# acoustid/acoustid-index

Measured on AMD Instinct MI355X. Metric: queries/sec + p50 /_search latency, 100M-fp index, 1k-hash queries, higher is better.
Workload: dtype u32

## Files before the change

acoustid-index_amd/csrc/fpx_qsearch.hpp:

```cpp
#pragma once
#include <hip/hip_runtime.h>

#include "fpx_internal.h"

namespace fpx {

#ifndef FPX_QS_WG
#define FPX_QS_WG 256
#endif
#ifndef FPX_QS_WAVES
#define FPX_QS_WAVES 4
#endif
#ifndef FPX_QS_REC_CAP
#define FPX_QS_REC_CAP 8192
#endif
#ifndef FPX_QS_FLOG2
#define FPX_QS_FLOG2 11
#endif
constexpr uint32_t QS_WG = FPX_QS_WG;
constexpr uint32_t QS_REC_CAP = FPX_QS_REC_CAP;
constexpr uint32_t QS_FLOG2 = FPX_QS_FLOG2;
constexpr uint32_t QS_TLOG2 = 8;
constexpr uint32_t QS_MAX_HASHES = QS_REC_CAP >= 8192u ? 4096u : 2048u;
constexpr uint32_t QS_MAX_ROUNDS = 32;
#ifndef FPX_QS_WORDS
#define FPX_QS_WORDS 12
#endif
#ifndef FPX_QS_CH
#define FPX_QS_CH 2
#endif
constexpr uint32_t QS_WORDS = FPX_QS_WORDS;
constexpr uint32_t QS_CH = FPX_QS_CH;
constexpr uint32_t QS_TASKS = (((size_t)2u << QS_FLOG2) + ((size_t)8u << QS_TLOG2)) / 8u;
constexpr uint32_t QS_TASK_WORDS = 8;
constexpr uint32_t QS_TASKS_FILT = QS_TASKS * 8u / 12u;
static_assert(QS_MAX_HASHES * 2u <= QS_REC_CAP, "the dedup set lives where the records will");
static_assert((QS_MAX_HASHES + QS_WG - 1u) / QS_WG <= QS_MAX_ROUNDS, "rounds per query");
static_assert(QS_WORDS % 4 == 0 && QS_WORDS <= 16, "the words are fetched in 16-byte pieces; a lane's masks of them are 16 bits");
#ifndef FPX_QS_DYN
#define FPX_QS_DYN 1
#endif
#ifndef FPX_QS_STAGGER
#define FPX_QS_STAGGER 1
#endif
constexpr uint32_t QS_STAGGER = FPX_QS_STAGGER;
#ifndef FPX_QS_WGS_PER_CU
#define FPX_QS_WGS_PER_CU 4
#endif
constexpr uint32_t QS_WGS_PER_CU = FPX_QS_WGS_PER_CU;
constexpr size_t QS_LDS_BYTES = ((size_t)QS_REC_CAP + 4u) * 4u + ((size_t)2u << QS_FLOG2) + ((size_t)8u << QS_TLOG2) + (size_t)SB_CAND * 8u;

struct QSearchArgs {
    const uint32_t* hashes_base; const uint64_t* offsets;
    const uint32_t* opts;
    uint32_t q_begin, q_end, sb;
    uint64_t* cands; uint64_t cand_cap;
    uint64_t* qcand; uint32_t* qcand_n;
    unsigned long long* counters;
    unsigned long long* stat_sets;
    unsigned long long* qstats;
    const uint32_t* cancel;
    const uint64_t* mem_tab; const uint32_t* mem_bucket; const uint32_t* mem_bits;
    unsigned int* next_q;
    uint32_t stagger;
    unsigned long long* redo; uint32_t redo_cap;
};

struct QSKernargs { QSearchArgs a; GroupArgs ga; };
typedef const __attribute__((address_space(4))) QSKernargs* qs_kargs_t;
__device__ __forceinline__ qs_kargs_t qs_cold_args()
{
    qs_kargs_t p = (qs_kargs_t)__builtin_amdgcn_kernarg_segment_ptr();
    asm volatile("" : "+s"(p));
    return p;
}

#define FPX_QS_OCC __attribute__((amdgpu_waves_per_eu(FPX_QS_WAVES)))
typedef uint32_t u32x3_t __attribute__((ext_vector_type(3)));
__device__ __forceinline__ uint3 gload_u3(const uint32_t* p)
{
    const u32x3_t v = *(const FPX_GLOBAL u32x3_t*)p;
    return make_uint3(v.x, v.y, v.z);
}
__device__ __forceinline__ uint32_t qs_cell(uint32_t doc) { return (doc ^ (doc >> QS_FLOG2)) & ((1u << QS_FLOG2) - 1u); }
__device__ __forceinline__ unsigned long long qs_task_list(const uint32_t* p, uint32_t chunk)
{
    return ((unsigned long long)p >> 2) | ((unsigned long long)chunk << 57) | (1ull << 63);
}
__device__ __forceinline__ unsigned long long qs_task_words(const uint32_t* p, uint32_t cnt, uint32_t second, uint32_t chunk)
{
    return ((unsigned long long)p >> 2) | ((unsigned long long)(cnt - 1u) << 46) | ((unsigned long long)(second & 0xFFu) << 49) | ((unsigned long long)chunk << 57);
}
__device__ __forceinline__ const uint32_t* qs_task_ptr(unsigned long long e) { return reinterpret_cast<const uint32_t*>((e & ((1ull << 46) - 1ull)) << 2); }
__device__ __forceinline__ uint32_t qs_word_cols(uint32_t pm, uint32_t dm, uint32_t j0, uint32_t cnt)
{
    uint32_t cols = 0, rest = pm, i = 0, w = 0;
    while (rest != 0u && w < j0 + cnt) {
        const uint32_t s = (uint32_t)__builtin_ctz(rest), span = 1u + ((dm >> i) & 1u);
        for (uint32_t t = 0; t < span; ++t, ++w) if (w >= j0 && w < j0 + cnt) cols |= s << (4u * (w - j0));
        ++i; rest &= rest - 1u;
    }
    return cols;
}

template <uint32_t K> __device__ __forceinline__ uint32_t qs_group_bcast(uint32_t v)
{
    return (uint32_t)__builtin_amdgcn_ds_swizzle((int)v, (int)((K << 5) | 0x18u));
}
template <uint32_t K> __device__ __forceinline__ uint32_t qs_from_sub0(uint32_t v)
{
    if constexpr (K == 0u) return v;
    else return (uint32_t)__builtin_amdgcn_update_dpp(0, (int)v, 0x110 | (int)K, 0xF, 0xF, true);
}
template <uint32_t K> __device__ __forceinline__ uint32_t qs_from_sub7(uint32_t v)
{
    if constexpr (K == 7u) return v;
    else return (uint32_t)__builtin_amdgcn_update_dpp(0, (int)v, 0x100 | (int)(7u - K), 0xF, 0xF, true);
}
template <uint32_t K> struct qs_idx { static constexpr uint32_t value = K; };
template <uint32_t K = 0, class F> __device__ __forceinline__ void qs_for8(F&& f)
{
    if constexpr (K < 8u) { f(qs_idx<K>{}); qs_for8<K + 1u>(f); }
}

#ifdef FPX_QS_PROF
#define QS_MARK(i) do { if (tid == 0) { const unsigned long long t_ = clock64(); atomicAdd(&qs_cold_args()->a.counters[CTR_HIST + (i)], t_ - t_prev); t_prev = t_; } } while (0)
#define QS_SUB0() do { if (tid == 0) t_sub = clock64(); } while (0)
#define QS_SUB(i) do { if (tid == 0) { const unsigned long long t_ = clock64(); atomicAdd(&qs_cold_args()->a.counters[CTR_HIST + (i)], t_ - t_sub); t_sub = t_; } } while (0)
#define QS_ARRIVED2(x, y) asm volatile("" :: "v"(x), "v"(y))
#define QS_ARRIVED4(x) asm volatile("" :: "v"((x)[0]), "v"((x)[1]), "v"((x)[2]), "v"((x)[3]))
#else
#define QS_MARK(i) do { } while (0)
#define QS_SUB0() do { } while (0)
#define QS_SUB(i) do { } while (0)
#define QS_ARRIVED2(x, y) do { } while (0)
#define QS_ARRIVED4(x) do { } while (0)
#endif
constexpr uint32_t QS_MAX_CLASSES = 32;
constexpr uint32_t QS_LIST_AHEAD = 8;
__device__ __forceinline__ uint32_t qs_class(uint32_t rec) { return mix32(rec) >> 27; }
static_assert(QS_MAX_CLASSES == 32u, "qs_class gives five bits");
constexpr uint32_t QS_LOW_CHUNK = 8;
template <int NS, bool QS, bool MEM, bool FILT, bool CLS, bool LOW = false, bool NEXT = false>
__device__ __forceinline__ void qs_body(const QSearchArgs& a, const GroupArgs& ga)
{
    static_assert(!NEXT || (!CLS && !LOW && !MEM), "a later group's walk: no doc classes, no low floors, no memory table (they ride on the first group's launch)");
    static_assert(!(CLS && FILT), "doc classes: the unfiltered walk only");
    static_assert(!LOW || (!CLS && QS_WG == 256u && QS_REC_CAP >= 512u && (QS_REC_CAP & (QS_REC_CAP - 1u)) == 0u),
                  "low floors: no doc classes; the sorted tail's scans are written for 256 lanes and a power-of-two array");
#ifdef FPX_QS_PROF
    unsigned long long t_prev = clock64(), t_sub = 0;
#endif
    constexpr uint32_t HVL = NS == 16 ? 2u : 3u;
    constexpr uint32_t T = 1u << QS_TLOG2, TMASK = T - 1u;
    extern __shared__ __align__(16) uint8_t qs_dyn[];
    uint32_t* const recs = reinterpret_cast<uint32_t*>(qs_dyn);
    uint32_t* const filter = recs + QS_REC_CAP + 4u;
    unsigned long long* const table = reinterpret_cast<unsigned long long*>(filter + (1u << (QS_FLOG2 - 1u)));
    unsigned long long* const tasks = reinterpret_cast<unsigned long long*>(filter);
    constexpr uint32_t TCAP = FILT ? QS_TASKS_FILT : QS_TASKS;
    uint32_t* const tcols = reinterpret_cast<uint32_t*>(tasks + QS_TASKS_FILT);
    uint64_t* const cbuf = reinterpret_cast<uint64_t*>(table + T);
    __shared__ uint32_t s_count, s_ntask, s_over_recs, s_seen_ones, s_cancel, s_claimed, s_full, s_ccnt, s_cshared, s_cbase_lo, s_cbase_hi;
    __shared__ unsigned long long wg_blocks, wg_docs, wg_probes, wg_reads;
    __shared__ uint32_t wg_h[HIST_SLOTS];
    __shared__ uint32_t s_first[FUSE_MAX], s_last[FUSE_MAX];
    __shared__ const uint32_t* s_ext[GROUP_CHUNKS];
    __shared__ uint32_t s_q2;
    __shared__ uint32_t s_dseg[FUSE_MAX];

    const uint32_t tid = threadIdx.x, lane = tid & 63u;
    const GroupDesc* g = &ga.g;
    uint32_t ent = a.q_begin + blockIdx.x;
    uint32_t q = ent, q_recs = 0u;
    uint32_t ncls = 1u;
    auto take_entry = [&]() {
        const unsigned long long e = qs_cold_args()->a.redo[ent];
        q = (uint32_t)__builtin_amdgcn_readfirstlane((int)(uint32_t)e); q_recs = (uint32_t)__builtin_amdgcn_readfirstlane((int)(uint32_t)(e >> 32));
        ncls = 1u;
        while ((unsigned long long)ncls * (QS_REC_CAP / 2u) < (unsigned long long)q_recs) ncls *= 2u;
    };
    if constexpr (CLS) take_entry();
    (void)q_recs;
    uint32_t qn = q + gridDim.x;
    uint32_t n, nn = 0u;
    uint64_t nq_lo = 0;
    const uint32_t* qh;
    if constexpr (CLS) {
        const uint64_t q_lo = a.offsets[q];
        n = (uint32_t)(a.offsets[q + 1] - q_lo);
        qh = a.hashes_base + q_lo;
        qn = 0xFFFFFFFFu;
    } else {
        const uint64_t q_lo = a.offsets[q];
        n = (uint32_t)(a.offsets[q + 1] - q_lo);
        qh = a.hashes_base + q_lo;
        if (qn < a.q_end) { nq_lo = a.offsets[qn]; nn = (uint32_t)(a.offsets[qn + 1] - nq_lo); }
    }
    {
        const qs_kargs_t ka = qs_cold_args();
        if (tid < FUSE_MAX) { s_first[tid] = ka->ga.g.first_hash[tid]; s_last[tid] = ka->ga.g.last_hash[tid]; }
        if (tid < GROUP_CHUNKS) s_ext[tid] = tid < ka->ga.g.nchunks ? ka->ga.g.ext_tab[tid] : nullptr;
        if (FILT && tid < FUSE_MAX) s_dseg[tid] = ka->ga.g.has_dead[tid] != 0u ? ka->ga.g.seg_index[tid] : 0xFFFFFFFFu;
    }
    const uint32_t gmin = (FILT || MEM) ? g->gmin : 0u;
    (void)gmin;
    uint32_t hq[2u * QS_CH];
    uint3 hd[QS_CH];
    auto line_of = [&](uint32_t h) -> const uint32_t* { return g->lines + (size_t)((h >> HVL) - g->line0) * GROUP_LINE_WORDS; };
    auto load_pair = [&](const uint32_t* qh_, uint32_t n_, uint32_t c, uint32_t& h0, uint32_t& h1) {
        const uint32_t i = c * QS_CH * QS_WG + tid;
        h0 = i < n_ ? gload_u32(qh_ + i) : 0u;
        h1 = i + QS_WG < n_ ? gload_u32(qh_ + i + QS_WG) : 0u;
    };
    auto issue_heads = [&](bool v0, bool v1) {
        hd[0] = gload_u3(v0 ? line_of(hq[0]) : g->lines);
        hd[1] = gload_u3(v1 ? line_of(hq[1]) : g->lines);
    };
    load_pair(qh, n, 0u, hq[0], hq[1]);
    load_pair(qh, n, 1u, hq[2], hq[3]);
    uint32_t c_host = 0u;
    unsigned long long c_dev = 0ull;
    auto ask_cancel = [&]() {
        const qs_kargs_t ka = qs_cold_args();
        const uint32_t* const cancel = ka->a.cancel;
        if (tid == 0u && cancel != nullptr) {
            if ((blockIdx.x & 63u) == 0u) c_host = __hip_atomic_load(cancel, __ATOMIC_RELAXED, __HIP_MEMORY_SCOPE_SYSTEM);
            c_dev = __hip_atomic_load(&ka->a.counters[CTR_CANCEL], __ATOMIC_RELAXED, __HIP_MEMORY_SCOPE_AGENT);
        }
    };
    ask_cancel();
  if (const uint32_t stagger = qs_cold_args()->a.stagger; !CLS && stagger != 0u && a.q_end - a.q_begin >= 4u * gridDim.x)
      for (uint32_t i = 0; i < ((blockIdx.x >> 8) & 3u) * stagger; ++i) __builtin_amdgcn_s_sleep(127);
  for (;;) {
    if constexpr (CLS) {
        if (ncls > QS_MAX_CLASSES) {
            if (tid == 0) atomicMax(&qs_cold_args()->a.counters[CTR_BINFAIL], 1ull);
            return;
        }
    }
    const uint32_t rounds = (n + QS_WG - 1u) / QS_WG, nchunks = (rounds + QS_CH - 1u) / QS_CH;
    uint32_t sbits = 8u;
    while ((1u << sbits) < 2u * n) ++sbits;
    if (tid < HIST_SLOTS) wg_h[tid] = 0u;
    for (uint32_t i = tid; i < (1u << sbits); i += QS_WG) recs[i] = 0xFFFFFFFFu;
    if (tid == 0) {
        s_count = 0u; s_ntask = 0u; s_over_recs = 0u; s_seen_ones = 0u; s_ccnt = 0u; s_cshared = 0u;
        wg_blocks = 0; wg_docs = 0; wg_probes = 0; wg_reads = 0;
        if (c_host != 0u) { atomicExch(&qs_cold_args()->a.counters[CTR_CANCEL], 1ull); c_dev = 1ull; }
        s_cancel = c_dev != 0ull ? 1u : 0u;
    }
    __syncthreads();
    if (s_cancel) return;
    QS_MARK(0);
    uint32_t vmask = 0u;
    uint32_t mmask = 0u;
    uint32_t nx[QS_CH] = {0u, 0u};
    for (uint32_t c = 0; c < nchunks; ++c) {
        uint32_t hc[QS_CH];
        uint32_t mb[QS_CH];
#pragma unroll
        for (uint32_t u = 0; u < QS_CH; ++u) hc[u] = c == 0u ? hq[u] : c == 1u ? hq[QS_CH + u] : nx[u];
        if (c != 0u) { QS_SUB0(); QS_ARRIVED2(hc[0], hc[1]); QS_SUB(6); }
        if (c != 0u && c + 1u < nchunks) load_pair(qh, n, c + 1u, nx[0], nx[1]);
        if constexpr (MEM) {
#pragma unroll
            for (uint32_t u = 0; u < QS_CH; ++u) {
                const uint32_t i = (c * QS_CH + u) * QS_WG + tid;
                mb[u] = (i < n && a.mem_bits != nullptr) ? gload_u32(a.mem_bits + ((hc[u] >> MEMTAB_FILTER_SHIFT) >> 5)) : 0xFFFFFFFFu;
            }
        }
#pragma unroll
        for (uint32_t u = 0; u < QS_CH; ++u) {
            const uint32_t i = (c * QS_CH + u) * QS_WG + tid;
            if (i >= n) continue;
            const uint32_t h = hc[u];
            bool dup;
            if (h == 0xFFFFFFFFu) dup = atomicExch(&s_seen_ones, 1u) != 0u;
            else {
                uint32_t slot = (h * 0x9E3779B1u) >> (32u - sbits);
                for (;;) {
                    const uint32_t old = atomicCAS(&recs[slot], 0xFFFFFFFFu, h);
                    if (old == 0xFFFFFFFFu) { dup = false; break; }
                    if (old == h) { dup = true; break; }
                    slot = (slot + 1u) & ((1u << sbits) - 1u);
                }
            }
            if (!dup && h >= g->win_lo && h <= g->win_hi) {
                vmask |= 1u << (c * QS_CH + u);
                if constexpr (MEM) mmask |= ((mb[u] >> ((h >> MEMTAB_FILTER_SHIFT) & 31u)) & 1u) << (c * QS_CH + u);
            }
        }
    }
    (void)mmask;
    __syncthreads();
    QS_MARK(1);

    const uint32_t cmask = ncls - 1u;
    (void)cmask;
    const bool has_next = qn < a.q_end;
    uint32_t q2 = 0u;
    bool has_q2 = false;
    uint64_t o2_lo = 0;
    uint32_t o2_hi = 0u;
  for (uint32_t cls = 0; cls < ncls; ++cls) {
    if constexpr (CLS) {
        if (cls != 0u) {
            __syncthreads();
            if (tid == 0) { s_count = 0u; s_ntask = 0u; }
            load_pair(qh, n, 0u, hq[0], hq[1]);
            __syncthreads();
        }
    }
    auto in_class = [&](uint32_t rec) -> bool { return (qs_class(rec) & cmask) == cls; };
    (void)in_class;
    const uint32_t active = g->active, nactive = (uint32_t)__popc(active);
    uint32_t my_blocks = 0, my_docs = 0, my_probes = 0, my_reads = 0;
    auto dead_in = [&](uint32_t s, uint32_t doc) -> bool {
        const uint32_t di = s_dseg[s];
        return di != 0xFFFFFFFFu && is_dead_seg(ga.segs[di], doc);
    };
    auto reserve_in = [&](uint32_t* counter, uint32_t cnt) -> uint32_t {
        const uint32_t incl = scan16(cnt);
        const uint32_t r0 = (uint32_t)__builtin_amdgcn_readlane((int)incl, 15), r1 = (uint32_t)__builtin_amdgcn_readlane((int)incl, 31),
                       r2 = (uint32_t)__builtin_amdgcn_readlane((int)incl, 47), r3 = (uint32_t)__builtin_amdgcn_readlane((int)incl, 63);
        const uint32_t total = r0 + r1 + r2 + r3;
        uint32_t wbase = 0;
        if (total != 0u) {
            if (lane == 0u) wbase = atomicAdd(counter, total);
            wbase = (uint32_t)__builtin_amdgcn_readfirstlane((int)wbase);
        }
        const uint32_t row = lane >> 4;
        return wbase + (row >= 1u ? r0 : 0u) + (row >= 2u ? r1 : 0u) + (row >= 3u ? r2 : 0u) + (incl - cnt);
    };
    auto reserve_both = [&](uint32_t cnt, uint32_t nt, uint32_t& tat) -> uint32_t {
        const uint32_t both = cnt | (nt << 16);
        const uint32_t incl = scan16(both);
        const uint32_t r0 = (uint32_t)__builtin_amdgcn_readlane((int)incl, 15), r1 = (uint32_t)__builtin_amdgcn_readlane((int)incl, 31),
                       r2 = (uint32_t)__builtin_amdgcn_readlane((int)incl, 47), r3 = (uint32_t)__builtin_amdgcn_readlane((int)incl, 63);
        const uint32_t total = r0 + r1 + r2 + r3;
        uint32_t rbase = 0, tbase = 0;
        if ((total & 0xFFFFu) != 0u) {
            if (lane == 0u) rbase = atomicAdd(&s_count, total & 0xFFFFu);
            rbase = (uint32_t)__builtin_amdgcn_readfirstlane((int)rbase);
        }
        if ((total >> 16) != 0u) {
            if (lane == 0u) tbase = atomicAdd(&s_ntask, total >> 16);
            tbase = (uint32_t)__builtin_amdgcn_readfirstlane((int)tbase);
        }
        const uint32_t row = lane >> 4;
        const uint32_t before = (row >= 1u ? r0 : 0u) + (row >= 2u ? r1 : 0u) + (row >= 3u ? r2 : 0u) + (incl - both);
        tat = tbase + (before >> 16);
        return rbase + (before & 0xFFFFu);
    };
    auto emit_at = [&](uint32_t km, const auto& d, uint32_t cnt, uint32_t pos) {
        constexpr uint32_t N = sizeof(d) / sizeof(uint32_t);
        if (cnt != 0u && pos + cnt > QS_REC_CAP) { s_over_recs = 1u; km = 0u; cnt = 0u; }
        const uint32_t first = cnt != 0u ? pos : QS_REC_CAP, sink = QS_REC_CAP - first;
#pragma unroll
        for (uint32_t j = N; j-- != 0u;) {
            const uint32_t last = (uint32_t)__popc(km & ((2u << j) - 1u)) - 1u;
            recs[first + min(last, sink)] = d[j];
        }
    };
    auto emit = [&](uint32_t km, const auto& d) {
        const uint32_t cnt = (uint32_t)__popc(km);
        emit_at(km, d, cnt, reserve_in(&s_count, cnt));
    };
    auto emit1 = [&](bool kp, uint32_t doc) {
        if constexpr (CLS) kp = kp && in_class(doc);
        const unsigned long long m = __ballot((int)kp);
        if (m == 0ull) return;
        uint32_t base = 0;
        if (lane == (uint32_t)__builtin_ctzll(m)) base = atomicAdd(&s_count, (uint32_t)__popcll(m));
        base = __shfl(base, (int)__builtin_ctzll(m));
        if (kp) {
            const uint32_t at = base + (uint32_t)__popcll(m & ((1ull << lane) - 1ull));
            if (at < QS_REC_CAP) recs[at] = doc; else s_over_recs = 1u;
        }
    };
    auto push_task = [&](unsigned long long e) {
        const uint32_t at = atomicAdd(&s_ntask, 1u);
        if (at < TCAP) tasks[at] = e; else s_over_recs = 1u;
    };

    auto words_of = [&](uint32_t h, uint3 head, bool valid, uint32_t (&gw)[QS_WORDS], uint32_t& hx, uint32_t& hy, uint32_t& ov) {
        const uint64_t bits = valid ? (((uint64_t)head.y << 32) | head.x) : 0ull;
        const uint32_t dfl = valid ? head.z : 0u;
        const uint32_t sh = (h & ((1u << HVL) - 1u)) * (uint32_t)NS;
        const uint32_t pm = (uint32_t)(bits >> sh) & ((1u << NS) - 1u);
        const uint32_t pos0 = (uint32_t)__popcll(bits & ((1ull << sh) - 1ull));
        const uint32_t k = (uint32_t)__popc(pm);
        const uint32_t dbl_before = pos0 >= 32u ? (uint32_t)__popc(dfl) : (uint32_t)__popc(dfl & ((1u << pos0) - 1u));
        const uint32_t dm = pos0 >= 32u ? 0u : ((dfl >> pos0) & ((1u << k) - 1u));
        const uint32_t nwords = k + (uint32_t)__popc(dm);
        const uint32_t n_line = (uint32_t)__popcll(bits) + (uint32_t)__popc(dfl);
        const uint32_t inl = n_line > GROUP_INLINE ? GROUP_INLINE - 1u : GROUP_INLINE;
        const uint32_t start = pos0 + dbl_before;
        const uint32_t mine = min(min(nwords, QS_WORDS), start < inl ? inl - start : 0u);
#pragma unroll
        for (uint32_t i = 0; i < QS_WORDS; ++i) gw[i] = 0xFFFFFFFFu;
        const uint32_t* lp = line_of(h) + 3u + start;
#pragma unroll
        for (uint32_t i = 0; i < QS_WORDS / 4; ++i) {
            if (mine > 4u * i) {
                const uint4 v = gload_u4_a4(lp + 4u * i);
                gw[4 * i] = v.x; gw[4 * i + 1] = v.y; gw[4 * i + 2] = v.z; gw[4 * i + 3] = v.w;
            }
        }
        ov = start + nwords > inl ? gload_u32(line_of(h) + (GROUP_LINE_WORDS - 1u)) : 0u;
        hx = start | (mine << 7) | (nwords << 11) | (inl << 17);
        hy = pm | (dm << 16);
    };
    auto probe = [&](uint32_t h, uint32_t hx, uint32_t hy, bool valid, uint32_t (&gw)[QS_WORDS], uint32_t ov) {
        if (valid) { my_probes += nactive; my_reads += 2u; }
        const uint32_t pm = hy & 0xFFFFu, dm = hy >> 16;
        const uint32_t start = hx & 127u, mine = (hx >> 7) & 15u, nwords = (hx >> 11) & 63u, inl = (hx >> 17) & 31u;
        uint32_t inr = active;
        if (h < g->lo_all || h > g->hi_all) {
            inr = 0u;
            uint32_t z = 0u;
            asm volatile("" : "+v"(z));
#pragma unroll
            for (uint32_t s = 0; s < NS; ++s) inr |= (h >= s_first[z + s] && h <= s_last[z + s]) ? (1u << s) : 0u;
        }
        if (!valid) inr = 0u;
        my_blocks += (uint32_t)__popc(inr & active & ~pm);
        uint32_t second = 0;
        for (uint32_t d = dm, t = 0; d != 0u; d &= d - 1u, ++t) second |= 1u << ((uint32_t)__builtin_ctz(d) + t + 1u);
        uint32_t negm = 0, gapm = 0;
#pragma unroll
        for (uint32_t j = 0; j < QS_WORDS; ++j) {
            const uint32_t word = gw[j];
            negm |= (word >> 31) << j;
            gapm |= (word == 0xFFFFFFFFu ? 1u : 0u) << j;
        }
        const uint32_t vm = (1u << mine) - 1u;
        uint32_t keep = vm & ~negm;
        uint32_t lmask = vm & negm & ~gapm;
        uint32_t dmask = 0;
        if constexpr (FILT) {
            uint32_t amask = 0;
            for (uint32_t r = pm, i = 0, w = 0; r != 0u && w < mine; r &= r - 1u, ++i) {
                const uint32_t s = (uint32_t)__builtin_ctz(r), span = 1u + ((dm >> i) & 1u), bits = ((1u << span) - 1u) << w;
                amask |= ((active >> s) & 1u) != 0u ? bits : 0u;
                dmask |= s_dseg[s] != 0xFFFFFFFFu ? bits : 0u;
                w += span;
            }
            keep &= amask; lmask &= amask;
        }
        my_docs += (uint32_t)__popc(keep);
        my_blocks += (uint32_t)__popc(keep & ~second);
        if constexpr (SCAN_HIST && (FPX_SH_BITS & 2)) my_probes += (uint32_t)__popc(keep & second) << 16;
        if constexpr (FILT) {
            for (uint32_t m = keep & dmask; m != 0u; m &= m - 1u) {
                const uint32_t j0 = (uint32_t)__builtin_ctz(m);
                uint32_t doc = 0;
#pragma unroll
                for (uint32_t j = 0; j < QS_WORDS; ++j) doc = j == j0 ? gw[j] : doc;
                if (dead_in(qs_word_cols(pm, dm, j0, 1u), gmin + doc)) keep &= ~(1u << j0);
            }
        }
        const uint32_t in_line = (nwords != mine && start + mine < inl) ? min(nwords - mine, inl - (start + mine)) : 0u;
        const uint32_t in_ext = nwords - mine - in_line;
        const uint32_t nt = (uint32_t)__popc(lmask) + (in_line + QS_TASK_WORDS - 1u) / QS_TASK_WORDS + (in_ext + QS_TASK_WORDS - 1u) / QS_TASK_WORDS;
        uint32_t tat;
        const uint32_t nrec = (uint32_t)__popc(keep);
        emit_at(keep, gw, nrec, reserve_both(nrec, nt, tat));
        if (nt != 0u) {
            if (tat + nt > TCAP) { s_over_recs = 1u; tat = TCAP; }
            auto put_task = [&](unsigned long long e) { if (tat < TCAP) tasks[tat] = e; ++tat; };
            auto put_words = [&](unsigned long long e, uint32_t j0, uint32_t c) {
                if constexpr (FILT) { if (tat < TCAP) tcols[tat] = qs_word_cols(pm, dm, j0, c); }
                put_task(e);
            };
            const uint32_t chunk = (h >> GROUP_CHUNK_LOG2) - g->chunk0;
            const uint32_t* ext = s_ext[chunk];
            uint32_t lm = lmask;
            while (lm != 0u) {
                const uint32_t j0 = (uint32_t)__builtin_ctz(lm);
                lm &= lm - 1u;
                uint32_t e = 0;
#pragma unroll
                for (uint32_t j = 0; j < QS_WORDS; ++j) e = j == j0 ? gw[j] : e;
                put_task(qs_task_list(ext + (e & 0x7FFFFFFFu), chunk) | (FILT ? ((unsigned long long)qs_word_cols(pm, dm, j0, 1u) << 46) : 0ull));
            }
            uint32_t j = mine;
            while (j < mine + in_line) {
                const uint32_t c = min(mine + in_line - j, QS_TASK_WORDS);
                put_words(qs_task_words(line_of(h) + 3u + start + j, c, second >> j, chunk), j, c);
                j += c;
            }
            if (j < nwords) {
                const uint32_t* ob = ext + ov;
                while (j < nwords) {
                    const uint32_t c = min(nwords - j, QS_TASK_WORDS);
                    put_words(qs_task_words(ob + (start + j - inl), c, second >> j, chunk), j, c);
                    j += c;
                }
                my_reads += 2u;
            }
        }
    };

    auto round_coop = [&](uint32_t h, bool valid) {
        const uint32_t sub = lane & 7u;
        uint32_t L[32];
        {
            const uint32_t li = valid ? (h >> HVL) - g->line0 : 0u;
            const uint8_t* const lb = reinterpret_cast<const uint8_t*>(g->lines) + 16u * sub;
            uint32_t lk[8];
            qs_for8([&](auto kc) { constexpr uint32_t k = decltype(kc)::value; lk[k] = qs_group_bcast<k>(li); });
            asm volatile("" : "+v"(lk[0]), "+v"(lk[1]), "+v"(lk[2]), "+v"(lk[3]), "+v"(lk[4]), "+v"(lk[5]), "+v"(lk[6]), "+v"(lk[7]));
            qs_for8([&](auto kc) {
                constexpr uint32_t k = decltype(kc)::value;
// ... 188 lines not shown
    QS_SUB0();
    QS_ARRIVED2(nn, (uint32_t)nq_lo); QS_SUB(11);
    uint32_t floor_v;
    {
        uint32_t qv = q;
        asm volatile("" : "+v"(qv));
        floor_v = gload_u32(qs_cold_args()->a.opts + (size_t)qv * 4u + 1u);
    }
    if (has_next) {
        const uint32_t* const qhn = a.hashes_base + nq_lo;
        load_pair(qhn, nn, 0u, hq[0], hq[1]);
        load_pair(qhn, nn, 1u, hq[2], hq[3]);
    }
    {
        uint32_t t_lo = 0;
        for (;;) {
            const uint32_t t_hi = min(s_ntask, TCAP);
            __syncthreads();
            if (t_lo >= t_hi) break;
            for (uint32_t t0 = t_lo; t0 < t_hi; t0 += QS_WG) {
                const bool has = t0 + tid < t_hi;
                const unsigned long long e = has ? tasks[t0 + tid] : 0ull;
                const bool is_list = has && (e >> 63) != 0ull;
                const uint32_t* p = qs_task_ptr(e);
                const uint32_t lcol = FILT ? (uint32_t)(e >> 46) & 15u : 0u;
                const uint32_t tc = (FILT && has && !is_list) ? tcols[t0 + tid] : 0u;
                uint32_t d[QS_TASK_WORDS];
#pragma unroll
                for (uint32_t j = 0; j < QS_TASK_WORDS; ++j) d[j] = 0xFFFFFFFFu;
                const uint32_t cnt = !has ? 0u : is_list ? 8u : ((uint32_t)(e >> 46) & 7u) + 1u;
#pragma unroll
                for (uint32_t i = 0; i < QS_TASK_WORDS / 4; ++i) {
                    if (cnt > 4u * i) {
                        const uint4 v = gload_u4_a4(p + 4u * i);
                        d[4 * i] = v.x; d[4 * i + 1] = v.y; d[4 * i + 2] = v.z; d[4 * i + 3] = v.w;
                    }
                }
                uint32_t km = 0, lm = 0;
                bool long_list = false;
                uint32_t eff = 0, Tl = 0, xin = 0;
                if (is_list) {
                    const uint32_t hdr = d[0];
                    eff = hdr & 0xFFFFu; Tl = (hdr >> 19) & 1u;
                    xin = min(eff, Tl ? 6u : 7u);
                    km = ((1u << xin) - 1u) << (1u + Tl);
                    my_blocks += (hdr >> 16) & 7u; my_docs += eff; my_reads += 2u;
                    hist_observe(wg_h, eff, (hdr >> 16) & 7u);
                    long_list = eff > xin;
                    if (long_list) my_reads += ((eff - xin + 31u) >> 5) * 2u;
                } else if (has) {
                    const uint32_t second = (uint32_t)(e >> 49) & 0xFFu;
                    uint32_t vm = (1u << cnt) - 1u, negm = 0, gapm = 0;
#pragma unroll
                    for (uint32_t j = 0; j < QS_TASK_WORDS; ++j) {
                        if constexpr (FILT) vm &= ~((((active >> ((tc >> (4u * j)) & 15u)) & 1u) ^ 1u) << j);
                        negm |= (d[j] >> 31) << j;
                        gapm |= (d[j] == 0xFFFFFFFFu ? 1u : 0u) << j;
                    }
                    km = vm & ~negm;
                    lm = vm & negm & ~gapm;
                    my_docs += (uint32_t)__popc(km); my_blocks += (uint32_t)__popc(km & ~second);
                    if constexpr (SCAN_HIST && (FPX_SH_BITS & 2)) my_probes += (uint32_t)__popc(km & second) << 16;
                }
                if constexpr (FILT) {
                    for (uint32_t m = km; m != 0u; m &= m - 1u) {
                        const uint32_t j0 = (uint32_t)__builtin_ctz(m);
                        const uint32_t s = is_list ? lcol : (tc >> (4u * j0)) & 15u;
                        if (s_dseg[s] == 0xFFFFFFFFu) continue;
                        uint32_t doc = 0;
#pragma unroll
                        for (uint32_t j = 0; j < QS_TASK_WORDS; ++j) doc = j == j0 ? d[j] : doc;
                        if (dead_in(s, gmin + doc)) km &= ~(1u << j0);
                    }
                }
                if constexpr (CLS) {
                    uint32_t cm = 0u;
#pragma unroll
                    for (uint32_t j = QS_TASK_WORDS; j-- != 0u;) cm = (cm << 1) | (in_class(d[j]) ? 1u : 0u);
                    km &= cm;
                }
                emit(km, d);
                while (lm != 0u) {
                    const uint32_t j0 = (uint32_t)__builtin_ctz(lm);
                    lm &= lm - 1u;
                    uint32_t w = 0;
#pragma unroll
                    for (uint32_t j = 0; j < QS_TASK_WORDS; ++j) w = j == j0 ? d[j] : w;
                    const uint32_t chunk = (uint32_t)(e >> 57) & 63u;
                    push_task(qs_task_list(s_ext[chunk] + (w & 0x7FFFFFFFu), chunk) | (FILT ? ((unsigned long long)((tc >> (4u * j0)) & 15u) << 46) : 0ull));
                }
                unsigned long long ml = __ballot((int)long_list);
                while (ml != 0ull) {
                    const int src = (int)__builtin_ctzll(ml);
                    ml &= ml - 1ull;
                    const uint32_t* list = reinterpret_cast<const uint32_t*>(((uint64_t)__shfl((uint32_t)((uint64_t)p >> 32), src) << 32) | __shfl((uint32_t)(uint64_t)p, src));
                    const uint32_t eff_s = __shfl(eff, src), T_s = __shfl(Tl, src), from = __shfl(xin, src);
                    const uint32_t col_s = FILT ? (uint32_t)__shfl(lcol, src) : 0u;
                    if constexpr (CLS) {
                        for (uint32_t o2 = from; o2 < eff_s; o2 += 64u * QS_LIST_AHEAD) {
                            uint32_t dv[QS_LIST_AHEAD];
#pragma unroll
                            for (uint32_t u = 0; u < QS_LIST_AHEAD; ++u)
                                dv[u] = o2 + 64u * u + lane < eff_s ? gload_u32(list + 1u + T_s + o2 + 64u * u + lane) : 0u;
#pragma unroll
                            for (uint32_t u = 0; u < QS_LIST_AHEAD; ++u) emit1(o2 + 64u * u + lane < eff_s, dv[u]);
                        }
                    } else
                    for (uint32_t o2 = from; o2 < eff_s; o2 += 64u) {
                        bool kp = o2 + lane < eff_s;
                        const uint32_t dv = kp ? gload_u32(list + 1u + T_s + o2 + lane) : 0u;
                        if constexpr (FILT) { if (kp) kp = !dead_in(col_s, gmin + dv); }
                        emit1(kp, dv);
                    }
                }
            }
            t_lo = t_hi;
            __syncthreads();
        }
    }

    for (uint32_t i = tid; i < (1u << (QS_FLOG2 - 1u)); i += QS_WG) filter[i] = 0u;
    for (uint32_t s = tid; s < T; s += QS_WG) table[s] = 0ull;
    {
        auto wave_total = [&](uint32_t v) -> unsigned long long {
            const uint32_t incl = scan16(v);
            return (unsigned long long)(uint32_t)__builtin_amdgcn_readlane((int)incl, 15) + (uint32_t)__builtin_amdgcn_readlane((int)incl, 31) +
                   (uint32_t)__builtin_amdgcn_readlane((int)incl, 47) + (uint32_t)__builtin_amdgcn_readlane((int)incl, 63);
        };
        const unsigned long long w_reads = wave_total(my_reads), w_blocks = wave_total(my_blocks), w_docs = wave_total(my_docs), w_probes = wave_total(my_probes & 0xFFFFu);
        const uint32_t w_doubles = (uint32_t)wave_total(my_probes >> 16);
        if (tid == 0u) s_q2 = qs_cold_args()->a.next_q != nullptr ? a.q_begin + 2u * gridDim.x + r2 : qn + gridDim.x;
        if (lane == 0u && (!CLS || cls == 0u)) {
            if (w_doubles) atomicAdd(&wg_h[0], w_doubles);
            if (w_reads) atomicAdd(&wg_reads, w_reads);
            if (w_blocks) atomicAdd(&wg_blocks, w_blocks);
            if (w_docs) atomicAdd(&wg_docs, w_docs);
            if (w_probes) atomicAdd(&wg_probes, w_probes);
        }
    }
    __syncthreads();
    QS_MARK(3);
    q2 = (uint32_t)__builtin_amdgcn_readfirstlane((int)s_q2);
    has_q2 = has_next && q2 < a.q_end;
    if (has_q2) {
        uint32_t qv = q2;
        asm volatile("" : "+v"(qv));
        o2_lo = gload_u64(a.offsets + qv); o2_hi = gload_u32(reinterpret_cast<const uint32_t*>(a.offsets + qv + 1u));
    }
    if (has_next) ask_cancel();
    const uint32_t nrec = min(s_count, QS_REC_CAP);
    for (uint32_t i = tid * 4u; i < nrec; i += QS_WG * 4u) {
        const uint4 r4 = *reinterpret_cast<const uint4*>(recs + i);
        const uint32_t r[4] = {r4.x, r4.y, r4.z, r4.w};
#pragma unroll
        for (uint32_t u = 0; u < 4u; ++u) {
            const uint32_t c = qs_cell(r[u]);
            if (i + u < nrec) atomicAdd(&filter[c >> 1], 1u << (16u * (c & 1u)));
        }
    }
    const qs_kargs_t kt = qs_cold_args();
    const bool q_stats = !CLS || cls == 0u;
    bool q_redo = false;
    if constexpr (!FILT && !CLS && !NEXT) {
        if (s_over_recs != 0u || s_count > QS_REC_CAP) q_redo = kt->a.redo != nullptr && s_ntask <= TCAP;
    }
    if (tid == 0 && q_redo) {
        const unsigned long long at = atomicAdd(&kt->a.counters[CTR_REDO], 1ull);
        if (at < (unsigned long long)kt->a.redo_cap) kt->a.redo[at] = (unsigned long long)q | ((unsigned long long)s_count << 32);
    }
    if (tid == 0 && !q_redo) {
        unsigned long long* st = kt->a.stat_sets + (size_t)(q % LEAN_STAT_SETS) * 8u;
        if (q_stats) {
            if (wg_reads) atomicAdd(&st[4], wg_reads);
            if (wg_blocks) atomicAdd(&st[1], wg_blocks);
            const uint32_t block_size = kt->ga.g.block_size;
            if (wg_blocks && block_size != 512u) atomicAdd(&st[5], wg_blocks * (unsigned long long)block_size - wg_blocks * 512ull);
            if (wg_docs) atomicAdd(&st[2], wg_docs);
            if (wg_probes) atomicAdd(&st[3], wg_probes);
        }
        if (s_count) atomicAdd(&st[7], (unsigned long long)s_count);
        if constexpr (QS && NEXT) { unsigned long long* const qstats = kt->a.qstats; if (qstats) qstats[q] += wg_blocks | (wg_docs << 32); }
        else if constexpr (QS) { if (q_stats) { unsigned long long* const qstats = kt->a.qstats; if (qstats) qstats[q] = wg_blocks | (wg_docs << 32); } }
        if (s_over_recs || s_count > QS_REC_CAP) atomicMax(&kt->a.counters[CTR_BINFAIL], 1ull);
    }
    if (tid < HIST_SLOTS - 1u && q_stats && !q_redo) {
        const unsigned long long v = tid == HIST_COUNT ? wg_probes : tid == HIST_DOCS ? wg_docs : tid == HIST_BLOCKS ? wg_blocks : (unsigned long long)wg_h[tid];
        if (v != 0ull) atomicAdd(&kt->a.stat_sets[(size_t)LEAN_STAT_SETS * 8u + (size_t)(q % LEAN_STAT_SETS) * HIST_SLOTS + tid], v);
    }
    const uint32_t floor_q = (uint32_t)__builtin_amdgcn_readfirstlane((int)floor_v);
    const uint32_t sb = kt->a.sb;
    const uint64_t smax = sb >= 32u ? 0xFFFFFFFFull : ((1ull << sb) - 1ull);
    const bool low_q = LOW && floor_q <= 2u;
    if constexpr (LOW) {
      if (low_q && s_over_recs == 0u && !q_redo && nrec != 0u && nrec >= floor_q && kt->a.opts[(size_t)q * 4u] != 0u) {
        const uint32_t kmax = kt->a.opts[(size_t)q * 4u], pct = kt->a.opts[(size_t)q * 4u + 2u];
        const uint32_t gmin_c = kt->ga.g.gmin;
        uint32_t* const lhist = filter;
        uint32_t* const lsc = filter + 256u;
        uint32_t P = 512u;
        while (P < nrec) P <<= 1;
        __syncthreads();
        for (uint32_t i = tid; i < P; i += QS_WG) recs[i] = i < nrec ? recs[i] + gmin_c : 0xFFFFFFFFu;
        lhist[tid] = 0u;
        if (tid < 8u) lsc[tid] = 0u;
        __syncthreads();
        auto cx = [](uint32_t& x, uint32_t& y, bool up) {
            const uint32_t lo = min(x, y), hi = max(x, y);
            x = up ? lo : hi; y = up ? hi : lo;
        };
        auto chunk_sort = [&](uint32_t k) {
            for (uint32_t c = tid; c < P / QS_LOW_CHUNK; c += QS_WG) {
                uint4* const at = reinterpret_cast<uint4*>(recs + c * QS_LOW_CHUNK);
                const uint4 x0 = at[0], x1 = at[1];
                uint32_t v[8] = {x0.x, x0.y, x0.z, x0.w, x1.x, x1.y, x1.z, x1.w};
                if (k == 0u) {
#pragma unroll
                    for (uint32_t kk = 2u; kk <= 8u; kk <<= 1)
#pragma unroll
                        for (uint32_t j = kk >> 1; j != 0u; j >>= 1)
#pragma unroll
                            for (uint32_t i = 0; i < 8u; ++i)
                                if ((i & j) == 0u) cx(v[i], v[i | j], kk == 8u ? (c & 1u) == 0u : (i & kk) == 0u);
                } else {
                    const bool up = ((c * QS_LOW_CHUNK) & k) == 0u;
#pragma unroll
                    for (uint32_t j = 4u; j != 0u; j >>= 1)
#pragma unroll
                        for (uint32_t i = 0; i < 8u; ++i)
                            if ((i & j) == 0u) cx(v[i], v[i | j], up);
                }
                at[0] = make_uint4(v[0], v[1], v[2], v[3]); at[1] = make_uint4(v[4], v[5], v[6], v[7]);
            }
        };
        static_assert(QS_LOW_CHUNK == 8u, "chunk_sort is written for eight places");
        chunk_sort(0u);
        __syncthreads();
        for (uint32_t k = 2u * QS_LOW_CHUNK; k <= P; k <<= 1) {
            for (uint32_t j = k >> 1; j >= QS_LOW_CHUNK; j >>= 1) {
                for (uint32_t w = tid; w < P / 8u; w += QS_WG) {
                    const uint32_t t0 = 4u * w, i = ((t0 & ~(j - 1u)) << 1) | (t0 & (j - 1u));
                    uint4* const pa = reinterpret_cast<uint4*>(recs + i);
                    uint4* const pb = reinterpret_cast<uint4*>(recs + i + j);
                    uint4 x = *pa, y = *pb;
                    const bool up = (i & k) == 0u;
                    cx(x.x, y.x, up); cx(x.y, y.y, up); cx(x.z, y.z, up); cx(x.w, y.w, up);
                    *pa = x; *pb = y;
                }
                __syncthreads();
            }
            chunk_sort(k);
            __syncthreads();
        }
        const uint32_t C = ((nrec + QS_WG - 1u) / QS_WG) | 1u;
        const uint32_t i0 = min(tid * C, nrec), i1 = min(i0 + C, nrec);
        auto run_len = [&](uint32_t i, uint32_t doc) -> uint32_t {
            if (i + 1u >= nrec || recs[i + 1u] != doc) return 1u;
            uint32_t lo = i + 2u, hi = nrec;
            while (lo < hi) {
                const uint32_t mid = (lo + hi) >> 1;
                if (recs[mid] == doc) lo = mid + 1u; else hi = mid;
            }
            return lo - i;
        };
        auto for_runs = [&](auto&& f) {
            uint32_t prev = (i0 != 0u && i0 < nrec) ? recs[i0 - 1u] : 0u;
            for (uint32_t i = i0; i < i1; ++i) {
                const uint32_t doc = recs[i];
                if (i == 0u || doc != prev) f(doc, run_len(i, doc));
                prev = doc;
            }
        };
        auto wave_incl = [&](uint32_t v) -> uint32_t {
            const uint32_t incl = scan16(v);
            const uint32_t r0 = (uint32_t)__builtin_amdgcn_readlane((int)incl, 15), r1 = (uint32_t)__builtin_amdgcn_readlane((int)incl, 31),
                           r2 = (uint32_t)__builtin_amdgcn_readlane((int)incl, 47);
            const uint32_t row = lane >> 4;
            return incl + (row >= 1u ? r0 : 0u) + (row >= 2u ? r1 : 0u) + (row >= 3u ? r2 : 0u);
        };
        {
            uint32_t ones = 0u, best = 0u;
            for_runs([&](uint32_t, uint32_t len) {
                best = max(best, len);
                if (len == 1u) ++ones; else atomicAdd(&lhist[min(len, 255u)], 1u);
            });
            if (ones != 0u) atomicAdd(&lhist[1], ones);
            if (best != 0u) atomicMax(&lsc[4], best);
        }
        __syncthreads();
        const uint32_t best_q = lsc[4];
        const uint32_t cut = max(floor_q, rel_floor(best_q, pct));
        if (best_q >= cut) {
            const uint32_t cb = min(cut, 255u);
            const uint32_t hm = tid >= cb ? lhist[tid] : 0u;
            const uint32_t wi = wave_incl(hm);
            if (lane == 63u) lsc[tid >> 6] = wi;
            __syncthreads();
            const uint32_t t0 = lsc[0], t1 = lsc[1], t2 = lsc[2], t3 = lsc[3], wv = tid >> 6;
            const uint32_t incl = wi + (wv >= 1u ? t0 : 0u) + (wv >= 2u ? t1 : 0u) + (wv >= 3u ? t2 : 0u);
            const uint32_t above = t0 + t1 + t2 + t3 - incl;
            if (above + hm >= kmax && above < kmax) {
                lsc[5] = tid == 255u ? 254u : tid;
                lsc[6] = tid == 255u ? 0u : kmax - above;
            }
            __syncthreads();
            const uint32_t tcut = lsc[5], quota = lsc[6];
            uint32_t rank = 0u;
            if (quota != 0u) {
                uint32_t mine = 0u;
                for_runs([&](uint32_t, uint32_t len) { mine += len == tcut ? 1u : 0u; });
                const uint32_t mi = wave_incl(mine);
                if (lane == 63u) lsc[tid >> 6] = mi;
                __syncthreads();
                rank = mi - mine + (wv >= 1u ? lsc[0] : 0u) + (wv >= 2u ? lsc[1] : 0u) + (wv >= 3u ? lsc[2] : 0u);
            }
            for_runs([&](uint32_t doc, uint32_t count) {
                if (count < cut || count < tcut) return;
                if (count == tcut && rank++ >= quota) return;
                if ((uint64_t)count > smax) atomicMax(&kt->a.counters[CTR_MAXSCORE], (unsigned long long)count);
                const uint64_t sc = (uint64_t)count > smax ? smax : (uint64_t)count;
                const uint64_t qpart = sb >= 32u ? 0ull : ((uint64_t)q << (32u + sb));
                const uint64_t key = qpart | ((smax - sc) << 32) | doc;
                const uint32_t at = atomicAdd(&s_ccnt, 1u);
                if (at < SB_CAND) cbuf[at] = key;
                else {
                    const unsigned long long gi = atomicAdd(&kt->a.counters[CTR_CANDS], 1ull);
                    if (gi < kt->a.cand_cap) kt->a.cands[gi] = key;
                    s_cshared = 1u;
                }
            });
        }
      }
    }
    if (!low_q && s_over_recs == 0u && !q_redo && nrec != 0u && nrec >= floor_q) {
        uint32_t passes = 1u;
        for (uint32_t pass = 0; pass < passes; ++pass) {
            if (pass != 0u) {
                __syncthreads();
                for (uint32_t s = tid; s < T; s += QS_WG) table[s] = 0ull;
            }
            if (tid == 0) { s_claimed = 0u; s_full = 0u; }
            __syncthreads();
            for (uint32_t i4 = tid * 4u; i4 < nrec; i4 += QS_WG * 4u) {
              const uint4 r4 = *reinterpret_cast<const uint4*>(recs + i4);
              const uint32_t r[4] = {r4.x, r4.y, r4.z, r4.w};
              uint32_t cnt4[4];
#pragma unroll
              for (uint32_t u = 0; u < 4u; ++u) { const uint32_t c = qs_cell(r[u]); cnt4[u] = (filter[c >> 1] >> (16u * (c & 1u))) & 0xFFFFu; }
#pragma unroll
              for (uint32_t u = 0; u < 4u; ++u) {
                const uint32_t doc = r[u];
                if (i4 + u >= nrec || cnt4[u] < floor_q) continue;
                const uint32_t h2 = mix32(doc);
                if (passes > 1u && (h2 >> 16) % passes != pass) continue;
                const unsigned long long keyhi = (unsigned long long)doc << 32;
                uint32_t s = h2 & TMASK;
                for (uint32_t tries = 0;; ++tries) {
                    if (tries == T) { s_full = 1u; break; }
                    unsigned long long cur = table[s];
                    if (cur == 0ull) {
                        const unsigned long long prev = atomicCAS(&table[s], 0ull, keyhi | 1ull);
                        if (prev == 0ull) { atomicAdd(&s_claimed, 1u); break; }
                        cur = prev;
                    }
                    if ((cur >> 32) == (keyhi >> 32)) { atomicAdd(&table[s], 1ull); break; }
                    s = (s + 1u) & TMASK;
                }
              }
            }
            __syncthreads();
            if (pass == 0u && (s_claimed > T * 3u / 4u || s_full != 0u) && passes < 64u) {
                const uint32_t np = passes * 2u;
                __syncthreads();
                for (uint32_t s = tid; s < T; s += QS_WG) table[s] = 0ull;
                passes = np; pass = 0xFFFFFFFFu;
                continue;
            }
            const qs_kargs_t kc = qs_cold_args();
            if (s_full != 0u && tid == 0) atomicMax(&kc->a.counters[CTR_BINFAIL], 1ull);
            const uint32_t gmin_c = kc->ga.g.gmin;
            for (uint32_t s = tid; s < T; s += QS_WG) {
                const unsigned long long e = table[s];
                if (e == 0ull) continue;
                const uint32_t count = (uint32_t)e, doc = gmin_c + (uint32_t)(e >> 32);
                if (count < floor_q) continue;
                if ((uint64_t)count > smax) atomicMax(&kc->a.counters[CTR_MAXSCORE], (unsigned long long)count);
                const uint64_t sc = (uint64_t)count > smax ? smax : (uint64_t)count;
                const uint64_t qpart = sb >= 32u ? 0ull : ((uint64_t)q << (32u + sb));
                const uint64_t key = qpart | ((smax - sc) << 32) | doc;
                const uint32_t at = atomicAdd(&s_ccnt, 1u);
                if (at < SB_CAND) cbuf[at] = key;
                else {
                    const unsigned long long gi = atomicAdd(&kc->a.counters[CTR_CANDS], 1ull);
                    if (gi < kc->a.cand_cap) kc->a.cands[gi] = key;
                    s_cshared = 1u;
                }
            }
        }
    }
  }
    __syncthreads();
    QS_MARK(4);
    const uint32_t cn = min(s_ccnt, SB_CAND);
    if constexpr (NEXT) {
        const qs_kargs_t kh = qs_cold_args();
        if (tid == 0) {
            uint32_t prev = kh->a.qcand_n[q];
            const bool was = prev == QCAND_OVERFLOWED;
            prev = was ? 0u : min(prev, QCAND_SLOTS);
            const bool to_slots = !was && s_cshared == 0u && prev + cn <= QCAND_SLOTS;
            if (!to_slots) {
                if (prev + cn != 0u) {
                    const unsigned long long gi = atomicAdd(&kh->a.counters[CTR_CANDS], (unsigned long long)(prev + cn));
                    s_cbase_lo = (uint32_t)gi; s_cbase_hi = (uint32_t)(gi >> 32);
                }
                if (!was) kh->a.qcand_n[q] = QCAND_OVERFLOWED;
            } else kh->a.qcand_n[q] = prev + cn;
            s_claimed = prev; s_full = to_slots ? 1u : 0u;
        }
        __syncthreads();
        const uint32_t prev = s_claimed;
        const bool to_slots = s_full != 0u;
        const uint64_t base = ((uint64_t)s_cbase_hi << 32) | s_cbase_lo;
        if (tid < cn) {
            const uint64_t key = cbuf[tid];
            if (to_slots) kh->a.qcand[(size_t)q * QCAND_SLOTS + prev + tid] = key;
            else if (base + tid < kh->a.cand_cap) kh->a.cands[base + tid] = key;
        }
        static_assert(SB_CAND + QCAND_SLOTS <= QS_WG, "the carried slots move by lanes of their own");
        if (const uint32_t t = tid - SB_CAND; !to_slots && t < prev) {
            const uint64_t gi = base + cn + t;
            if (gi < kh->a.cand_cap) kh->a.cands[gi] = kh->a.qcand[(size_t)q * QCAND_SLOTS + t];
        }
    } else {
    const bool shared = s_cshared != 0u || cn > QCAND_SLOTS;
    const qs_kargs_t kh = qs_cold_args();
    if (tid == 0) {
        if (shared && cn != 0u) {
            const unsigned long long gi = atomicAdd(&kh->a.counters[CTR_CANDS], (unsigned long long)cn);
            s_cbase_lo = (uint32_t)gi; s_cbase_hi = (uint32_t)(gi >> 32);
        }
        kh->a.qcand_n[q] = shared ? QCAND_OVERFLOWED : cn;
    }
    __syncthreads();
    if (tid < cn) {
        const uint64_t key = cbuf[tid];
        if (!shared) kh->a.qcand[(size_t)q * QCAND_SLOTS + tid] = key;
        else {
            const uint64_t gi = (((uint64_t)s_cbase_hi << 32) | s_cbase_lo) + tid;
            if (gi < kh->a.cand_cap) kh->a.cands[gi] = key;
        }
    }
    }
    QS_MARK(5);
    if constexpr (CLS) {
        ent += gridDim.x;
        if (ent >= a.q_end) break;
        take_entry();
        const uint64_t q_lo = a.offsets[q];
        n = (uint32_t)(a.offsets[q + 1] - q_lo);
        qh = a.hashes_base + q_lo;
        load_pair(qh, n, 0u, hq[0], hq[1]);
        load_pair(qh, n, 1u, hq[2], hq[3]);
        ask_cancel();
    } else {
        if (!has_next) break;
        q = qn; n = nn; qh = a.hashes_base + nq_lo;
        qn = q2; nn = 0u; nq_lo = 0;
        if (has_q2) {
            nq_lo = ((uint64_t)(uint32_t)__builtin_amdgcn_readfirstlane((int)(uint32_t)(o2_lo >> 32)) << 32) | (uint32_t)__builtin_amdgcn_readfirstlane((int)(uint32_t)o2_lo);
            nn = (uint32_t)__builtin_amdgcn_readfirstlane((int)(o2_hi - (uint32_t)o2_lo));
        }
    }
    __syncthreads();
  }
}

template <int NS, bool QS, bool MEM, bool FILT>
__global__ __launch_bounds__(QS_WG) FPX_QS_OCC void k_search_query(QSearchArgs a, GroupArgs ga)
{
    qs_body<NS, QS, MEM, FILT, false>(a, ga);
}

template <int NS, bool MEM>
__global__ __launch_bounds__(QS_WG) FPX_QS_OCC void k_search_classes(QSearchArgs a, GroupArgs ga)
{
    qs_body<NS, true, MEM, false, true>(a, ga);
}

template <int NS, bool QS, bool MEM>
__global__ __launch_bounds__(QS_WG) FPX_QS_OCC void k_search_low(QSearchArgs a, GroupArgs ga)
{
    qs_body<NS, QS, MEM, false, false, true>(a, ga);
}

template <int NS, bool QS, bool MEM>
__global__ __launch_bounds__(QS_WG) FPX_QS_OCC void k_search_low_filt(QSearchArgs a, GroupArgs ga)
{
    qs_body<NS, QS, MEM, true, false, true>(a, ga);
}

template <int NS, bool QS, bool FILT>
__global__ __launch_bounds__(QS_WG) FPX_QS_OCC void k_search_next(QSearchArgs a, GroupArgs ga)
{
    qs_body<NS, QS, false, FILT, false, false, true>(a, ga);
}

__global__ __launch_bounds__(256) void k_qs_zero(unsigned long long* counters, unsigned int* words, uint32_t nwords)
{
    const uint32_t i0 = blockIdx.x * 256u + threadIdx.x;
    if (i0 < CTR_COUNT) counters[i0] = 0ull;
    for (uint32_t i = i0; i < nwords; i += gridDim.x * 256u) words[i] = 0u;
}

}
```

Baseline: 27.00 million.

## Precompute per-lane survivor bitmask and compact hash-table inserts across lanes

Before the counting-table passes, each lane now reads its records and filter counts once and packs a survivor bitmask (up to 8 turns of 4 records). The insert loop then walks only the set bits, so lanes stay busy on real survivors instead of diverging on filtered records, and passes after the first skip the filter lookups. The change also splits off the full-vector case in the filter-build and emit paths and casts the record pointer to LDS address space so the compiler emits ds instructions. It adds a bitmask limit tied to REC_CAP and restructures the pass-reset synchronisation, which could introduce subtle ordering bugs.

```diff
diff --git a/acoustid-index_amd/csrc/fpx_qsearch.hpp b/acoustid-index_amd/csrc/fpx_qsearch.hpp
--- a/acoustid-index_amd/csrc/fpx_qsearch.hpp
+++ b/acoustid-index_amd/csrc/fpx_qsearch.hpp
@@ -76,6 +76,7 @@
 }
 
 #define FPX_QS_OCC __attribute__((amdgpu_waves_per_eu(FPX_QS_WAVES)))
+#define FPX_LDS __attribute__((address_space(3)))
 typedef uint32_t u32x3_t __attribute__((ext_vector_type(3)));
 __device__ __forceinline__ uint3 gload_u3(const uint32_t* p)
 {
@@ -357,10 +358,14 @@
         constexpr uint32_t N = sizeof(d) / sizeof(uint32_t);
         if (cnt != 0u && pos + cnt > QS_REC_CAP) { s_over_recs = 1u; km = 0u; cnt = 0u; }
         const uint32_t first = cnt != 0u ? pos : QS_REC_CAP, sink = QS_REC_CAP - first;
-#pragma unroll
-        for (uint32_t j = N; j-- != 0u;) {
-            const uint32_t last = (uint32_t)__popc(km & ((2u << j) - 1u)) - 1u;
-            recs[first + min(last, sink)] = d[j];
+        auto last_of = [&](uint32_t j) -> uint32_t { return (uint32_t)__popc(km & ((2u << j) - 1u)) - 1u; };
+        if constexpr (CLS) {
+#pragma unroll
+            for (uint32_t j = N; j-- != 0u;) recs[first + min(last_of(j), sink)] = d[j];
+        } else {
+            FPX_LDS uint32_t* const base = (FPX_LDS uint32_t*)(recs + first);
+#pragma unroll
+            for (uint32_t j = N; j-- != 0u;) base[min(last_of(j), sink)] = d[j];
         }
     };
     auto emit = [&](uint32_t km, const auto& d) {
@@ -855,10 +860,18 @@
     for (uint32_t i = tid * 4u; i < nrec; i += QS_WG * 4u) {
         const uint4 r4 = *reinterpret_cast<const uint4*>(recs + i);
         const uint32_t r[4] = {r4.x, r4.y, r4.z, r4.w};
-#pragma unroll
-        for (uint32_t u = 0; u < 4u; ++u) {
-            const uint32_t c = qs_cell(r[u]);
-            if (i + u < nrec) atomicAdd(&filter[c >> 1], 1u << (16u * (c & 1u)));
+        if (i + 3u < nrec) {
+#pragma unroll
+            for (uint32_t u = 0; u < 4u; ++u) {
+                const uint32_t c = qs_cell(r[u]);
+                atomicAdd(&filter[c >> 1], 1u << (16u * (c & 1u)));
+            }
+        } else {
+#pragma unroll
+            for (uint32_t u = 0; u < 4u; ++u) {
+                const uint32_t c = qs_cell(r[u]);
+                if (i + u < nrec) atomicAdd(&filter[c >> 1], 1u << (16u * (c & 1u)));
+            }
         }
     }
     const qs_kargs_t kt = qs_cold_args();
@@ -1035,47 +1048,60 @@
       }
     }
     if (!low_q && s_over_recs == 0u && !q_redo && nrec != 0u && nrec >= floor_q) {
+        if (tid == 0) { s_claimed = 0u; s_full = 0u; }
+        __syncthreads();
+        static_assert((QS_REC_CAP + QS_WG * 4u - 1u) / (QS_WG * 4u) <= 8u, "a lane's turns over a query's records: at most 8, four bits of its mask each");
+        uint32_t surv = 0u;
+        uint32_t t4 = tid * 4u;
+        asm volatile("" : "+v"(t4));
+        for (uint32_t i4 = t4, sh = 0u; i4 < nrec; i4 += QS_WG * 4u, sh += 4u) {
+            const uint4 r4 = *reinterpret_cast<const uint4*>(recs + i4);
+            const uint32_t r[4] = {r4.x, r4.y, r4.z, r4.w};
+            uint32_t cnt4[4];
+#pragma unroll
+            for (uint32_t u = 0; u < 4u; ++u) { const uint32_t c = qs_cell(r[u]); cnt4[u] = (filter[c >> 1] >> (16u * (c & 1u))) & 0xFFFFu; }
+            uint32_t m4 = 0u;
+            if (i4 + 3u < nrec) {
+#pragma unroll
+                for (uint32_t u = 0; u < 4u; ++u) m4 |= (cnt4[u] >= floor_q ? 1u : 0u) << u;
+            } else {
+#pragma unroll
+                for (uint32_t u = 0; u < 4u; ++u) m4 |= (i4 + u < nrec && cnt4[u] >= floor_q ? 1u : 0u) << u;
+            }
+            surv |= m4 << sh;
+        }
         uint32_t passes = 1u;
         for (uint32_t pass = 0; pass < passes; ++pass) {
-            if (pass != 0u) {
+            for (uint32_t left = surv; __ballot((int)(left != 0u)) != 0ull;) {
+                if (left != 0u) {
+                    const uint32_t bit = (uint32_t)__builtin_ctz(left);
+                    left &= left - 1u;
+                    const uint32_t doc = recs[(bit >> 2) * (QS_WG * 4u) + t4 + (bit & 3u)];
+                    const uint32_t h2 = mix32(doc);
+                    if (passes == 1u || (h2 >> 16) % passes == pass) {
+                        const unsigned long long keyhi = (unsigned long long)doc << 32;
+                        uint32_t s = h2 & TMASK;
+                        for (uint32_t tries = 0;; ++tries) {
+                            if (tries == T) { s_full = 1u; break; }
+                            unsigned long long cur = table[s];
+                            if (cur == 0ull) {
+                                const unsigned long long prev = atomicCAS(&table[s], 0ull, keyhi | 1ull);
+                                if (prev == 0ull) { atomicAdd(&s_claimed, 1u); break; }
+                                cur = prev;
+                            }
+                            if ((cur >> 32) == (keyhi >> 32)) { atomicAdd(&table[s], 1ull); break; }
+                            s = (s + 1u) & TMASK;
+                        }
+                    }
+                }
+            }
+            __syncthreads();
+            if (pass == 0u && (s_claimed > T * 3u / 4u || s_full != 0u) && passes < 64u) {
                 __syncthreads();
                 for (uint32_t s = tid; s < T; s += QS_WG) table[s] = 0ull;
-            }
-            if (tid == 0) { s_claimed = 0u; s_full = 0u; }
-            __syncthreads();
-            for (uint32_t i4 = tid * 4u; i4 < nrec; i4 += QS_WG * 4u) {
-              const uint4 r4 = *reinterpret_cast<const uint4*>(recs + i4);
-              const uint32_t r[4] = {r4.x, r4.y, r4.z, r4.w};
-              uint32_t cnt4[4];
-#pragma unroll
-              for (uint32_t u = 0; u < 4u; ++u) { const uint32_t c = qs_cell(r[u]); cnt4[u] = (filter[c >> 1] >> (16u * (c & 1u))) & 0xFFFFu; }
-#pragma unroll
-              for (uint32_t u = 0; u < 4u; ++u) {
-                const uint32_t doc = r[u];
-                if (i4 + u >= nrec || cnt4[u] < floor_q) continue;
-                const uint32_t h2 = mix32(doc);
-                if (passes > 1u && (h2 >> 16) % passes != pass) continue;
-                const unsigned long long keyhi = (unsigned long long)doc << 32;
-                uint32_t s = h2 & TMASK;
-                for (uint32_t tries = 0;; ++tries) {
-                    if (tries == T) { s_full = 1u; break; }
-                    unsigned long long cur = table[s];
-                    if (cur == 0ull) {
-                        const unsigned long long prev = atomicCAS(&table[s], 0ull, keyhi | 1ull);
-                        if (prev == 0ull) { atomicAdd(&s_claimed, 1u); break; }
-                        cur = prev;
-                    }
-                    if ((cur >> 32) == (keyhi >> 32)) { atomicAdd(&table[s], 1ull); break; }
-                    s = (s + 1u) & TMASK;
-                }
-              }
-            }
-            __syncthreads();
-            if (pass == 0u && (s_claimed > T * 3u / 4u || s_full != 0u) && passes < 64u) {
-                const uint32_t np = passes * 2u;
+                if (tid == 0) { s_claimed = 0u; s_full = 0u; }
+                passes *= 2u; pass = 0xFFFFFFFFu;
                 __syncthreads();
-                for (uint32_t s = tid; s < T; s += QS_WG) table[s] = 0ull;
-                passes = np; pass = 0xFFFFFFFFu;
                 continue;
             }
             const qs_kargs_t kc = qs_cold_args();
@@ -1098,6 +1124,12 @@
                     s_cshared = 1u;
                 }
             }
+            if (pass + 1u < passes) {
+                __syncthreads();
+                for (uint32_t s = tid; s < T; s += QS_WG) table[s] = 0ull;
+                if (tid == 0) { s_claimed = 0u; s_full = 0u; }
+                __syncthreads();
+            }
         }
     }
   }
```

Result: faster. 28.87 million, median of 6 (+6.9%).
